# pouyaardehkhani/4DLangSplat

Hardware: AMD Instinct MI355X
Metric: rasterizer fwd+bwd frames/sec @ 2M Gaussians, 1352x1014, 32-ch features (higher is better)
Workload: dtype f32; 1 GPU; S2M synthetic (BASELINE configs[2] per GPU; configs[3] batch split); gaussians=2000000, width=1352, height=1014, channels=32, global_batch=8, parallelism=dp1, pipeline=batched, binning=sort, early_views=2, order_on_side=True, num_rendered_mean=5615889

## Files before the change

4dlangsplat_amd/csrc/binning.hip:

```cpp
#include "lsr_common.h"
#include "lsr_internal.h"

namespace lsr {

__global__ void __launch_bounds__(256) k_emit(const EmitBatch eb) {
    __shared__ uint32_t s_off[4][64];
    __shared__ uint2 s_rc[4][64];
    __shared__ uint32_t s_id[4][64];
    __shared__ EmitSplat s_sp[4][64];
    const EmitView& ev = eb.v[blockIdx.y];
    const int P = eb.P, gx = eb.grid_x, W = eb.W, H = eb.H;
    const uint32_t* __restrict__ order = ev.order;
    const uint32_t* __restrict__ offsets = ev.offsets;
    const uint32_t* __restrict__ counts = ev.counts;
    const uint2* __restrict__ rect_sorted = ev.rect_sorted;
    const float2* __restrict__ xy = ev.xy;
    const float4* __restrict__ conic_o = ev.conic_o;
    uint32_t* __restrict__ keys = ev.keys;
    uint32_t* __restrict__ vals = ev.vals;
    clear_words(ev.clear);
    const int w = threadIdx.x >> 6, lane = threadIdx.x & 63;
    const int base = (blockIdx.x * 4 + w) * 64;
    if (base >= P) return;
    const int r = base + lane;
// ... 20 lines not shown
            if (s_off[w][k + step] <= j) k += step;
        const uint2 rc = s_rc[w][k];
        uint32_t x0, y0, x1, y1;
        rect_unpack(rc, x0, y0, x1, y1);
        const uint32_t wd = x1 - x0;
        const uint32_t loc = j - s_off[w][k];
        uint32_t dx, dy, quads;
        if (rect_small(x0, y0, x1, y1)) {
            const uint32_t map = rect_quad_map(rc);
            uint32_t m = rect_tile_mask(map);
            for (uint32_t i = 0; i < loc; ++i) m &= m - 1u;
            const uint32_t pos = (uint32_t)__builtin_ctz(m);
            dx = pos & 1u;
            dy = pos >> 1;
            const uint32_t sh = 8 * dy + 2 * dx;
            quads = ((map >> sh) & 3u) | (((map >> (sh + 4)) & 3u) << 2);
        } else {
            dy = loc / wd;
            dx = loc - dy * wd;
            quads = emit_quad_mask(s_sp[w][k], (int)(x0 + dx) * LSR_TILE_X, (int)(y0 + dy) * LSR_TILE_Y, W, H);
        }
        const uint32_t tx = x0 + dx, ty = y0 + dy;
        keys[j] = quads ? ty * (uint32_t)gx + tx : 0xFFFFFFFFu;
        vals[j] = s_id[w][k] | (quads << PL_QUAD_SHIFT);
    }
}

void launch_emit_instances(const EmitBatch& eb, int nv, hipStream_t st) {
    if (eb.P == 0 || nv <= 0) return;
    hipLaunchKernelGGL(k_emit, dim3((eb.P + 255) / 256, nv), dim3(256), 0, st, eb);
}

__global__ void __launch_bounds__(256) k_scatter_inst_off(int P, const uint32_t* __restrict__ order,
                                                          const uint32_t* __restrict__ offsets,
                                                          const uint32_t* __restrict__ counts,
                                                          uint32_t* __restrict__ inst_off) {
    const int r = blockIdx.x * blockDim.x + threadIdx.x;
    if (r < P && counts[r] > 0) inst_off[order[r]] = offsets[r];
}

void launch_scatter_inst_off(int P, const uint32_t* order, const uint32_t* offsets, const uint32_t* counts,
                             uint32_t* inst_off, hipStream_t st) {
    if (P == 0) return;
    hipLaunchKernelGGL(k_scatter_inst_off, dim3((P + 255) / 256), dim3(256), 0, st, P, order, offsets, counts,
                       inst_off);
}

}
```

4dlangsplat_amd/csrc/lsr_api.hip:

```cpp
#include <hip/hip_runtime.h>

#include <atomic>
#include <cstdio>
#include <cstring>
#include <mutex>
#include <string>
#include <vector>

#include "../../include/lsr.h"
#include "lsr_common.h"
#include "lsr_internal.h"

namespace {

thread_local std::string g_err;
std::atomic<int32_t> g_caller_api{0};

int fail(int code, const std::string& msg) {
    g_err = msg;
    return code;
}

#define LSR_HIP(expr)                                                                        \
    do {                                                                                     \
// ... 40 lines not shown
    ~PhaseTimer() {
        if (!a || !b) return;
        (void)hipEventRecord(b, st);
        std::lock_guard<std::mutex> l(g_prof.mu);
        g_prof.pending.push_back({phase, a, b});
    }
};

constexpr size_t kAlign = 256;
inline size_t al(size_t x) { return (x + kAlign - 1) / kAlign * kAlign; }

struct Carver {
    char* base;
    size_t off = 0;
    explicit Carver(void* b) : base(static_cast<char*>(b)) {}
    template <typename T>
    T* take(size_t n) {
        T* p = base ? reinterpret_cast<T*>(base + off) : nullptr;
        off += al(n * sizeof(T));
        return p;
    }
};

struct Geom {
    float2* xy;
    float4* conic_o;
    float4* rgbd;
    uint8_t* clamped;
    uint32_t* tiles;
    uint32_t *key_a, *key_b, *val_a, *val_b;
    uint32_t* counts;
    uint32_t* offsets;
    uint32_t* inst_off;
    int* radius;
    uint2* rect;
    uint2* rect_sorted;
    uint32_t* total;
    void* sort_tmp;
    void* scan_tmp;
    float4* acc;
};
Geom carve_geom(void* base, size_t P, size_t* bytes) {
    Carver c(base);
    Geom g;
    g.xy = c.take<float2>(P);
    g.conic_o = c.take<float4>(P);
    g.rgbd = c.take<float4>(P);
    g.clamped = c.take<uint8_t>(P);
    g.tiles = c.take<uint32_t>(P);
    g.key_a = c.take<uint32_t>(P);
    g.key_b = c.take<uint32_t>(P);
    g.val_a = c.take<uint32_t>(P);
    g.val_b = c.take<uint32_t>(P);
    g.counts = c.take<uint32_t>(P);
    g.offsets = c.take<uint32_t>(P);
    g.inst_off = c.take<uint32_t>(P);
    g.radius = c.take<int>(P);
    g.rect = c.take<uint2>(P);
    g.rect_sorted = c.take<uint2>(P);
    g.total = c.take<uint32_t>(4);
    g.sort_tmp = c.take<char>(lsr::radix_temp_bytes(P));
    g.scan_tmp = c.take<char>(lsr::scan_temp_bytes(P));
    g.acc = c.take<float4>(P * (lsr::ACC_PITCH / 4));
    if (bytes) *bytes = c.off;
    return g;
}

struct Binning {
    uint32_t *key_a, *key_b, *val_a, *val_b;
    void* sort_tmp;
    uint32_t* kept;
};
Binning carve_binning(void* base, size_t K, size_t* bytes) {
    Carver c(base);
    Binning b;
    b.key_a = c.take<uint32_t>(K);
    b.key_b = c.take<uint32_t>(K);
    b.val_a = c.take<uint32_t>(K);
    b.val_b = c.take<uint32_t>(K);
    b.sort_tmp = c.take<char>(lsr::radix_temp_bytes(K));
    b.kept = c.take<uint32_t>(4);
    if (bytes) *bytes = c.off;
    return b;
}

struct BinningTb {
    Binning b;
    uint32_t* table;
    uint64_t* tmp;
};
// ... 120 lines not shown
        if (!rules.share_first && !shares(s[v], s[0], rules.share)) return fail(LSR_EINVAL, rules.share_msg);
    }
    return LSR_OK;
}
int need_radii(int32_t n_views, lsr_fwd_out* const* out, int P) {
    for (int v = 0; v < n_views; ++v)
        if (!out[v] || (!out[v]->radii && P > 0)) return fail(LSR_EINVAL, "radii output is required");
    return LSR_OK;
}
int need_workspaces(const void* geom, const void* img, const void* binning, int64_t num_rendered) {
    if (!geom || !img || (num_rendered > 0 && !binning)) return fail(LSR_EINVAL, "workspaces are required");
    return LSR_OK;
}
int need_atomic_grads(const lsr_bwd_in* gin, const char* color_msg, const char* deterministic_msg) {
    if (!gin || !gin->dL_dout_color) return fail(LSR_EINVAL, color_msg);
    if (gin->deterministic) return fail(LSR_EINVAL, deterministic_msg);
    return LSR_OK;
}

void preprocess_shared(lsr::PreprocessArgs& a, const lsr_settings* s, const lsr_fwd_in* in) {
    const int W = s->image_width, H = s->image_height;
    const Grid grid = tile_grid(W, H);
    a.P = in->P; a.M = in->M; a.deg = s->sh_degree; a.W = W; a.H = H;
    a.grid_x = grid.x; a.grid_y = grid.y;
    a.scale_modifier = s->scale_modifier;
    a.means3D = in->means3D; a.scales = in->scales; a.rotations = in->rotations; a.opacities = in->opacities;
    a.shs = in->shs; a.colors_precomp = in->colors_precomp; a.cov3D_precomp = in->cov3D_precomp;
}
void preprocess_view(lsr::PreprocessView& v, const lsr_settings* s, const Geom& g, int* radii) {
    v.tanfovx = s->tanfovx; v.tanfovy = s->tanfovy;
    v.focal_x = focal(s->image_width, s->tanfovx);
    v.focal_y = focal(s->image_height, s->tanfovy);
    v.view = s->viewmatrix; v.proj = s->projmatrix; v.campos = s->campos;
    v.radii = radii; v.radius = g.radius; v.tiles = g.tiles; v.rect = g.rect; v.key = g.key_a; v.xy = g.xy;
    v.conic_o = g.conic_o; v.rgbd = g.rgbd; v.clamped = g.clamped;
    v.order = g.val_a;
    v.rank_counts = g.counts;
    v.acc = g.acc;
    v.clear.p[0] = g.total;
    v.clear.n[0] = 4;
}

uint32_t* mapped_counts(uint32_t* host_counts) {
    void* dptr = nullptr;
    if (hipHostGetDevicePointer(&dptr, host_counts, 0) == hipSuccess && dptr) return static_cast<uint32_t*>(dptr);
    (void)hipGetLastError();
    return nullptr;
}

int scan_counts(int nv, void* const* geom, int P, uint32_t* host_counts, uint32_t* mapped, hipStream_t st, bool debug) {
    lsr::ScanSeg sc[lsr::LSR_MAX_VIEWS] = {};
    const uint32_t* total[lsr::LSR_MAX_VIEWS];
    for (int k = 0; k < nv; ++k) {
        Geom g = carve_geom(geom[k], (size_t)P, nullptr);
        sc[k] = lsr::ScanSeg{g.counts, g.offsets, g.total, reinterpret_cast<uint32_t*>(g.scan_tmp), (size_t)P};
        total[k] = g.total;
        if (mapped) {
            sc[k].host_total = mapped + 2 * k;
            host_counts[2 * k + 1] = 0;
        }
    }
    uint32_t wrote;
    {
        PhaseTimer t(LSR_PHASE_INSTANCE_SCAN, st);
        wrote = lsr::exclusive_scan_batch(sc, nv, st);
    }
    LSR_LAUNCHED("instance scan", st, debug);
    for (int k = 0; k < nv; ++k)
        if (!((wrote >> k) & 1u))
// ... 66 lines not shown
    if (row1 == row0) return LSR_OK;
    for (int v0 = 0; v0 < n_views; v0 += lsr::LSR_MAX_VIEWS) {
        const int nv = std::min(n_views - v0, lsr::LSR_MAX_VIEWS);
        lsr::PreprocessArgs a{};
        preprocess_shared(a, s[v0], in);
        a.nv = nv;
        a.row0 = row0;
        a.P = row1;
        a.counts_tiles = counts_tiles;
        for (int k = 0; k < nv; ++k) {
            Geom g = carve_geom(geom[v0 + k], (size_t)P, nullptr);
            preprocess_view(a.v[k], s[v0 + k], g, out[v0 + k]->radii);
        }
        {
            PhaseTimer t(LSR_PHASE_PREPROCESS, st);
            lsr::launch_preprocess(a, st);
        }
        LSR_LAUNCHED("preprocess", st, s[v0]->debug);
    }
    return LSR_OK;
}

int depth_order_views(int32_t n_views, const lsr_settings* const* s, const lsr_fwd_in* in, void* const* geom,
                      uint32_t* host_counts, uint32_t* mapped, hipStream_t st) {
    const int P = in->P;
    for (int v0 = 0; v0 < n_views; v0 += lsr::LSR_MAX_VIEWS) {
        const int nv = std::min(n_views - v0, lsr::LSR_MAX_VIEWS);
        lsr::SortSeg ss[lsr::LSR_MAX_VIEWS] = {};
        for (int k = 0; k < nv; ++k) {
            Geom g = carve_geom(geom[v0 + k], (size_t)P, nullptr);
            ss[k] = lsr::SortSeg{g.key_a, g.val_a, g.key_b, g.val_b, g.sort_tmp, g.total + 3,
                                 lsr::SortGather{g.rect, g.counts, g.rect_sorted}, (size_t)P};
            ss[k].vals_c = g.offsets;
        }
        {
            PhaseTimer t(LSR_PHASE_DEPTH_SORT, st);
            if (lsr::radix_sort_batch(ss, nv, 0, 32, st) != depth_sort_result_in_b())
                return fail(LSR_EHIP, "internal: depth sort batch or parity");
        }
        LSR_LAUNCHED("depth sort", st, s[v0]->debug);
        int rc = scan_counts(nv, geom + v0, P, host_counts + 2 * v0, mapped ? mapped + 2 * v0 : nullptr, st,
                             s[v0]->debug);
        if (rc) return rc;
    }
    return LSR_OK;
}

int instance_scan_views(int32_t n_views, const lsr_fwd_in* in, void* const* geom, uint32_t* host_counts,
                        uint32_t* mapped, hipStream_t st, bool debug) {
    for (int v0 = 0; v0 < n_views; v0 += lsr::LSR_MAX_VIEWS) {
        int rc = scan_counts(std::min(n_views - v0, lsr::LSR_MAX_VIEWS), geom + v0, in->P, host_counts + 2 * v0,
                             mapped ? mapped + 2 * v0 : nullptr, st, debug);
        if (rc) return rc;
    }
    return LSR_OK;
}
}
}

namespace {
int preprocess_and_order(int32_t n_views, int32_t n_ordered, const lsr_settings* const* s, const lsr_fwd_in* in,
                         lsr_fwd_out* const* out, void* const* geom, uint32_t* host_counts, bool map_counts,
                         hipStream_t st) {
    if (in->P == 0) {
        for (int v = 0; v < 2 * n_ordered; ++v) host_counts[v] = 0;
        return LSR_OK;
// ... 129 lines not shown
    LSR_HIP(hipStreamSynchronize(reinterpret_cast<hipStream_t>(stream)));
    *num_rendered = (int64_t)tot[0];
    return LSR_OK;
}

int lsr_forward_binning(const lsr_settings* s, const lsr_fwd_in* in, void* geom, void* binning, void* img,
                        int64_t num_rendered, lsr_stream_t stream) {
    return lsr_forward_binning_views(1, &s, in, &geom, &binning, &img, &num_rendered, stream);
}

int lsr_forward_binning_views(int32_t n_views, const lsr_settings* const* s, const lsr_fwd_in* in, void* const* geom,
                              void* const* binning, void* const* img, const int64_t* num_rendered,
                              lsr_stream_t stream) {
    const auto emit_and_sort = [](const BinBatch& c, const BinView* bv, int ne) {
        const size_t ntiles = c.ntiles;
        hipStream_t st = c.st;
        lsr::EmitBatch eb{};
        eb.P = c.P; eb.grid_x = c.grid.x; eb.grid_y = c.grid.y; eb.W = c.W; eb.H = c.H;
        lsr::SortSeg ss[lsr::LSR_MAX_VIEWS] = {};
        for (int k = 0; k < ne; ++k) {
            const Geom& g = bv[k].g;
            const Img& m = bv[k].m;
            Binning b = carve_binning(bv[k].binning, bv[k].K, nullptr);
            lsr::EmitView& e = eb.v[k];
            e.order = g.val_a; e.offsets = g.offsets; e.counts = g.counts; e.rect_sorted = g.rect_sorted;
            e.xy = g.xy; e.conic_o = g.conic_o; e.keys = b.key_a; e.vals = b.val_a;
            e.clear.p[0] = reinterpret_cast<uint32_t*>(m.ranges);
            e.clear.n[0] = (uint32_t)(2 * ntiles);
            e.clear.even[0] = 0xFFFFFFFFu;
            e.clear.p[1] = m.tile_max;
            e.clear.n[1] = (uint32_t)ntiles;
            ss[k] = lsr::SortSeg{b.key_a, b.val_a, b.key_b, b.val_b, b.sort_tmp, b.kept,
                                 lsr::SortGather{nullptr, nullptr, nullptr}, bv[k].K, m.ranges, (uint32_t)ntiles};
        }
        {
            PhaseTimer t(LSR_PHASE_EMIT, st);
            lsr::launch_emit_instances(eb, ne, st);
        }
        LSR_LAUNCHED("emit", st, c.debug);
        {
            PhaseTimer t(LSR_PHASE_TILE_SORT, st);
            const int in_b = lsr::radix_sort_batch(ss, ne, 0, tile_bits((int)ntiles), st);
            if (in_b < 0 || (in_b == 1) != tile_sort_in_b((int)ntiles))
                return fail(LSR_EHIP, "internal: tile sort batch or parity");
        }
        LSR_LAUNCHED("tile sort", st, c.debug);
        return LSR_OK;
    };
    return bin_views(n_views, s, in, geom, binning, img, num_rendered, stream, SIZE_MAX, nullptr, emit_and_sort);
}

int lsr_forward_binning_views_tb(int32_t n_views, const lsr_settings* const* s, const lsr_fwd_in* in, void* const* geom,
                                 void* const* binning, void* const* img, const int64_t* num_rendered,
                                 lsr_stream_t stream) {
    const auto bucket = [](const BinBatch& c, const BinView* bv, int ne) {
        lsr::TbBatch tb{};
        tb.P = c.P; tb.grid_x = c.grid.x; tb.grid_y = c.grid.y; tb.W = c.W; tb.H = c.H; tb.ntiles = (int)c.ntiles;
        for (int k = 0; k < ne; ++k) {
            const Geom& g = bv[k].g;
            const Img& m = bv[k].m;
            BinningTb b = carve_binning_tb(bv[k].binning, bv[k].K, (size_t)c.P, c.ntiles, nullptr);
            lsr::TbView& t = tb.v[k];
            t.counts = g.counts; t.offsets = g.offsets; t.rect = g.rect; t.xy = g.xy; t.conic_o = g.conic_o;
            t.depth = g.key_a;
            t.table = b.table;
            t.tile_total = m.tile_order;
// ... 75 lines not shown
    lsr::launch_language_split(P, language_feature, out, reinterpret_cast<hipStream_t>(stream));
    LSR_LAUNCHED("language split", reinterpret_cast<hipStream_t>(stream), false);
    return LSR_OK;
}

int lsr_forward_render(const lsr_settings* s, const lsr_fwd_in* in, lsr_fwd_out* out, void* geom, void* binning,
                       void* img, int64_t num_rendered, lsr_stream_t stream) {
    if (!out || !out->out_color || !out->out_depth) return fail(LSR_EINVAL, "color and depth outputs are required");
    int rc = lsr_forward_binning(s, in, geom, binning, img, num_rendered, stream);
    if (rc) return rc;
    return lsr_forward_composite(s, in, out, geom, binning, img, num_rendered, stream);
}

int lsr_backward(const lsr_settings* s, const lsr_fwd_in* in, const lsr_bwd_in* gin, lsr_bwd_out* gout,
                 const void* geom, const void* binning, const void* img, void* scratch, int64_t num_rendered,
                 int32_t accumulate, lsr_stream_t stream) {
    int rc = check_common(s, in);
    if (rc) return rc;
    if (!gin || !gin->dL_dout_color || !gout) return fail(LSR_EINVAL, "dL_dout_color and outputs are required");
    if (!geom || !img || !scratch || (num_rendered > 0 && !binning)) return fail(LSR_EINVAL, "workspaces are required");
    hipStream_t st = reinterpret_cast<hipStream_t>(stream);
    const int P = in->P, W = s->image_width, H = s->image_height, C = in->C;
    if (P == 0) return LSR_OK;
    const size_t K = (size_t)num_rendered;
    Geom g = carve_geom(const_cast<void*>(geom), (size_t)P, nullptr);
    Binning b = carve_binning(const_cast<void*>(binning), K > 0 ? K : 1, nullptr);
    Img m = carve_img(const_cast<void*>(img), W, H, nullptr);
    const int Ceff = s->include_feature ? C : 0;
    const int recq = lsr::record_floats(Ceff);
    const bool det = gin->deterministic != 0;
    Scratch sc = carve_scratch(scratch, (size_t)P, K > 0 ? K : 1, recq, det, nullptr);
    if (det && K > 0) {
        LSR_HIP(hipMemsetAsync(sc.flags, 0, K, st));
        lsr::launch_scatter_inst_off(P, g.val_a, g.offsets, g.counts, g.inst_off, st);
    }
    if (!det) LSR_HIP(hipMemsetAsync(sc.acc_small, 0, sizeof(float) * lsr::ACC_PITCH * (size_t)P, st));
    if (!accumulate && C > 0 && gout->dL_dlanguage_feature && (!det || Ceff == 0))
        LSR_HIP(hipMemsetAsync(gout->dL_dlanguage_feature, 0, sizeof(float) * (size_t)P * C, st));
    if (K > 0) {
        lsr::RenderBwdArgs r{};
        render_bwd_view(r, s, in, gin, g, b, m);
        r.rec = sc.rec; r.flags = sc.flags; r.recq = recq; r.deterministic = det;
        r.acc_small = sc.acc_small; r.acc_lang = gout->dL_dlanguage_feature;
        {
            PhaseTimer t(LSR_PHASE_RENDER_BWD, st);
            lsr::launch_render_bwd(r, st);
        }
        LSR_LAUNCHED("render backward", st, s->debug);
    }
    lsr::PreprocessBwdArgs a{};
    a.P = P; a.M = in->M; a.deg = s->sh_degree;
    a.tanfovx = s->tanfovx; a.tanfovy = s->tanfovy;
    a.focal_x = focal(W, s->tanfovx);
    a.focal_y = focal(H, s->tanfovy);
    a.scale_modifier = s->scale_modifier;
    a.means3D = in->means3D; a.scales = in->scales; a.rotations = in->rotations; a.shs = in->shs;
    a.cov3D_precomp = in->cov3D_precomp; a.view = s->viewmatrix; a.proj = s->projmatrix; a.campos = s->campos;
    a.tiles = g.tiles;
    a.clamped = g.clamped;
    a.rec = sc.rec; a.flags = sc.flags; a.inst_off = g.inst_off; a.recq = recq;
    a.deterministic = det; a.acc_small = sc.acc_small;
    a.dopacity = gout->dL_dopacity;
    a.dmeans3D = gout->dL_dmeans3D; a.dmeans2D = gout->dL_dmeans2D; a.dcolors = gout->dL_dcolors;
    a.dcov3D = gout->dL_dcov3D; a.dsh = in->shs ? gout->dL_dsh : nullptr; a.dscales = gout->dL_dscales;
    a.drots = gout->dL_drotations;
    {
        PhaseTimer t(LSR_PHASE_PREPROCESS_BWD, st);
// ... 208 lines not shown
```

4dlangsplat_amd/csrc/lsr_internal.h:

```cpp
#pragma once
#include <hip/hip_runtime.h>
#include <stdint.h>

namespace lsr {

constexpr int ACC_PITCH = 16;

struct ClearList {
    uint32_t* p[4];
    uint32_t n[4];
    uint32_t even[4];
};

constexpr int LSR_MAX_VIEWS = 8;
__device__ __forceinline__ void clear_words(const ClearList& c) {
    const uint32_t t = blockIdx.x * blockDim.x + threadIdx.x, stride = gridDim.x * blockDim.x;
#pragma unroll
    for (int k = 0; k < 4; ++k)
        for (uint32_t i = t; i < c.n[k]; i += stride) c.p[k][i] = (i & 1u) ? 0u : c.even[k];
}

__host__ __device__ __forceinline__ uint2 rect_pack(uint32_t x0, uint32_t y0, uint32_t x1, uint32_t y1, uint32_t map) {
    return make_uint2(x0 | y0 << 12 | (map & 0xFFu) << 24, x1 | y1 << 12 | (map >> 8) << 24);
}
__host__ __device__ __forceinline__ void rect_unpack(uint2 r, uint32_t& x0, uint32_t& y0, uint32_t& x1, uint32_t& y1) {
    x0 = r.x & 0xFFFu; y0 = (r.x >> 12) & 0xFFFu; x1 = r.y & 0xFFFu; y1 = (r.y >> 12) & 0xFFFu;
}
__host__ __device__ __forceinline__ uint32_t rect_quad_map(uint2 r) { return (r.x >> 24) | (r.y >> 24) << 8; }
__host__ __device__ __forceinline__ bool rect_small(uint32_t x0, uint32_t y0, uint32_t x1, uint32_t y1) {
    return x1 - x0 <= 2 && y1 - y0 <= 2;
}
__host__ __device__ __forceinline__ uint32_t rect_tile_mask(uint32_t map) {
    return ((map & 0x33u) ? 1u : 0u) | ((map & 0xCCu) ? 2u : 0u) | ((map & 0x3300u) ? 4u : 0u) |
           ((map & 0xCC00u) ? 8u : 0u);
}
__host__ __device__ __forceinline__ uint32_t rect_count(uint2 r) {
    uint32_t x0, y0, x1, y1;
    rect_unpack(r, x0, y0, x1, y1);
    if ((x1 - x0) * (y1 - y0) > 0 && rect_small(x0, y0, x1, y1)) return __builtin_popcount(rect_tile_mask(rect_quad_map(r)));
    return (x1 - x0) * (y1 - y0);
}
__host__ __device__ __forceinline__ uint32_t rect_local_index(uint2 r, uint32_t tx, uint32_t ty) {
    uint32_t x0, y0, x1, y1;
    rect_unpack(r, x0, y0, x1, y1);
    if (rect_small(x0, y0, x1, y1))
        return __builtin_popcount(rect_tile_mask(rect_quad_map(r)) & ((1u << (2 * (ty - y0) + (tx - x0))) - 1u));
    return (ty - y0) * (x1 - x0) + (tx - x0);
}

struct PreprocessView {
    float tanfovx, tanfovy, focal_x, focal_y;
    const float* view;
    const float* proj;
    const float* campos;
    int* radii;
    int* radius;
    uint32_t* tiles;
    uint2* rect;
    uint32_t* key;
    float2* xy;
    float4* conic_o;
    float4* rgbd;
    uint8_t* clamped;
    uint32_t* order;
    uint32_t* rank_counts;
    float4* acc;
    ClearList clear;
};
struct PreprocessArgs {
    int P, M, deg, W, H, grid_x, grid_y, nv;
    int row0;
    int counts_tiles;
    float scale_modifier;
    const float* means3D;
    const float* scales;
    const float* rotations;
    const float* opacities;
    const float* shs;
    const float* colors_precomp;
    const float* cov3D_precomp;
    PreprocessView v[LSR_MAX_VIEWS];
};

struct PreprocessBwdArgs {
    int P, M, deg;
    float tanfovx, tanfovy, focal_x, focal_y, scale_modifier;
    const float* means3D;
    const float* scales;
    const float* rotations;
    const float* shs;
    const float* cov3D_precomp;
    const float* view;
    const float* proj;
    const float* campos;
    const uint32_t* tiles;
    const uint8_t* clamped;
    const float* rec;
// ... 242 lines not shown
void launch_preprocess_bwd(const PreprocessBwdArgs& a, bool accumulate, hipStream_t st);
void launch_reduce_lang(int P, int C, int cpad, int recq, const float* rec, const uint8_t* flags,
                        const uint32_t* inst_off, const uint32_t* tiles, float* dlang, bool accumulate, hipStream_t st);
void launch_mark_visible(int P, const float* means3D, const float* view, uint8_t* present, hipStream_t st);

size_t scan_temp_bytes(size_t n);
void exclusive_scan_u32(const uint32_t* in, uint32_t* out, size_t n, uint32_t* total, void* temp, hipStream_t st);
constexpr int SCAN_SEG_TILES = 4096;
struct ScanSeg {
    const uint32_t* in;
    uint32_t* out;
    uint32_t* total;
    uint32_t* partials;
    size_t n;
    uint32_t* host_total = nullptr;
};
struct ScanBatch { ScanSeg s[LSR_MAX_VIEWS]; };
uint32_t exclusive_scan_batch(const ScanSeg* segs, int nseg, hipStream_t st);
size_t radix_temp_bytes(size_t n);
struct SortGather {
    const uint2* rect;
    uint32_t* counts;
    uint2* rect_sorted;
};
struct SortSeg {
    uint32_t *keys_a, *vals_a, *keys_b, *vals_b;
    void* temp;
    uint32_t* kept;
    SortGather gather;
    size_t n;
    uint2* ranges;
    uint32_t nranges;
    uint32_t* vals_c;
};
struct SortBatch { SortSeg s[LSR_MAX_VIEWS]; };
int radix_sort_batch(const SortSeg* segs, int nseg, int begin_bit, int end_bit, hipStream_t st);
bool radix_sort_pairs(uint32_t* keys_a, uint32_t* vals_a, uint32_t* keys_b, uint32_t* vals_b, size_t n,
                      int begin_bit, int end_bit, void* temp, hipStream_t st, uint32_t* kept = nullptr,
                      const SortGather* gather = nullptr, uint32_t* vals_c = nullptr);

constexpr uint32_t PL_ID_MASK = 0x0FFFFFFFu;
constexpr int PL_QUAD_SHIFT = 28;
struct EmitView {
    const uint32_t* order;
    const uint32_t* offsets;
    const uint32_t* counts;
    const uint2* rect_sorted;
    const float2* xy;
    const float4* conic_o;
    uint32_t* keys;
    uint32_t* vals;
    ClearList clear;
};
struct EmitBatch {
    int P, grid_x, grid_y, W, H;
    EmitView v[LSR_MAX_VIEWS];
};
void launch_emit_instances(const EmitBatch& eb, int nv, hipStream_t st);
void launch_scatter_inst_off(int P, const uint32_t* order, const uint32_t* offsets, const uint32_t* counts,
                             uint32_t* inst_off, hipStream_t st);
struct TbView {
    const uint32_t* counts;
    const uint32_t* offsets;
    const uint2* rect;
    const float2* xy;
    const float4* conic_o;
    const uint32_t* depth;
    uint32_t* table;
    uint32_t* tile_total;
    uint32_t* tile_start;
    uint2* ranges;
    uint64_t* keys;
    uint64_t* tmp;
    uint32_t* words;
    uint32_t* tile_max;
};
struct TbBatch {
    int P, grid_x, grid_y, W, H, ntiles;
    TbView v[LSR_MAX_VIEWS];
};
int tb_blocks(int P);
hipError_t launch_tile_bucket_binning(const TbBatch& tb, int nv, hipStream_t st);

void launch_render_bwd(const RenderBwdArgs& a, hipStream_t st);
void launch_render_fwd_wave_views(const RenderFwdArgs* a, int n, hipStream_t st);
void launch_render_fwd_wave_mfma_views(const RenderFwdArgs* a, int n, hipStream_t st);

}
```

4dlangsplat_amd/csrc/preprocess.hip:

```cpp
#include "lsr_common.h"
#include "lsr_internal.h"

namespace lsr {

struct m3 { float m[3][3]; };

__device__ __forceinline__ m3 mul(const m3& a, const m3& b) {
    m3 o;
#pragma unroll
    for (int c = 0; c < 3; ++c)
#pragma unroll
        for (int r = 0; r < 3; ++r)
            o.m[c][r] = a.m[0][r] * b.m[c][0] + a.m[1][r] * b.m[c][1] + a.m[2][r] * b.m[c][2];
    return o;
}
__device__ __forceinline__ m3 tr(const m3& a) {
    m3 o;
#pragma unroll
    for (int c = 0; c < 3; ++c)
#pragma unroll
        for (int r = 0; r < 3; ++r) o.m[c][r] = a.m[r][c];
    return o;
}
__device__ __forceinline__ m3 quat_R(float4 q) {
// ... 73 lines not shown
#pragma unroll
        for (int k = 0; k < 6; ++k) c3[k] = a.cov3D_precomp[6 * (size_t)i + k];
    } else {
        const float3 s = make_float3(a.scales[3 * i], a.scales[3 * i + 1], a.scales[3 * i + 2]);
        const float4 q = reinterpret_cast<const float4*>(a.rotations)[i];
        cov3d(s, a.scale_modifier, q, c3);
    }
}
template <int MS, int N>
__device__ __forceinline__ void load_sh(const PreprocessArgs& a, int i, float (&shr)[N]) {
    constexpr int M3 = MS * 3;
    const float* src = a.shs + (size_t)i * M3;
    if (M3 % 4 == 0 && (reinterpret_cast<uintptr_t>(src) & 15) == 0) {
#pragma unroll
        for (int q = 0; q < M3 / 4; ++q) {
            const float4 t = reinterpret_cast<const float4*>(src)[q];
            shr[4 * q] = t.x; shr[4 * q + 1] = t.y; shr[4 * q + 2] = t.z; shr[4 * q + 3] = t.w;
        }
    } else {
#pragma unroll
        for (int q = 0; q < M3; ++q) shr[q] = src[q];
    }
}
template <int MS>
__device__ __forceinline__ void load_gauss(const PreprocessArgs& a, int i, GaussIn<MS>& g) {
    g.p = load_mean(a, i);
    g.op = a.opacities[i];
    load_cov3d(a, i, g.c3);
    if constexpr (MS > 0) {
        if (a.shs && !a.colors_precomp) load_sh<MS>(a, i, g.sh);
    }
}

template <int MS, bool PRE>
__device__ __forceinline__ bool preprocess_one(const PreprocessArgs& a, const PreprocessView& v, const GaussIn<MS>& g,
                                               int i) {
    v.radii[i] = 0;
    v.radius[i] = 0;
    v.tiles[i] = 0;
    v.rect[i] = make_uint2(0u, 0u);
    v.clamped[i] = 0;
    if (v.order) v.order[i] = (uint32_t)i;
    if (v.rank_counts) v.rank_counts[i] = 0u;
    if (v.key) v.key[i] = 0xFFFFFFFFu;
    const float3 p = PRE ? g.p : load_mean(a, i);
    const float4 ph = xform4x4(v.proj, p);
    const float3 pv = xform4x3(v.view, p);
    if (pv.z <= 0.2f) return false;
    const float pw = 1.0f / (ph.w + 0.0000001f);
    const float3 pp = make_float3(ph.x * pw, ph.y * pw, ph.z * pw);

    float c3[6];
    if constexpr (PRE) {
#pragma unroll
        for (int k = 0; k < 6; ++k) c3[k] = g.c3[k];
    } else {
        load_cov3d(a, i, c3);
    }
    float3 t = pv;
    const float limx = 1.3f * v.tanfovx, limy = 1.3f * v.tanfovy;
    const float txtz = t.x / t.z, tytz = t.y / t.z;
    t.x = fminf(limx, fmaxf(-limx, txtz)) * t.z;
    t.y = fminf(limy, fmaxf(-limy, tytz)) * t.z;
    m3 J = zero3();
    J.m[0][0] = v.focal_x / t.z; J.m[0][2] = -(v.focal_x * t.x) / (t.z * t.z);
    J.m[1][1] = v.focal_y / t.z; J.m[1][2] = -(v.focal_y * t.y) / (t.z * t.z);
    const m3 T = mul(view_W(v.view), J);
    const m3 V = sym3(c3);
    const m3 A = mul(tr(T), tr(V));
    const m3 cv = mul(A, T);
    const float ca = cv.m[0][0] + 0.3f, cb = cv.m[0][1], cc = cv.m[1][1] + 0.3f;
    const float det = ca * cc - cb * cb;
    if (det == 0.0f) return false;
    const float det_inv = 1.0f / det;
    const float4 conic = make_float4(cc * det_inv, -cb * det_inv, ca * det_inv, PRE ? g.op : a.opacities[i]);
    const float mid = 0.5f * (ca + cc);
    const float l1 = mid + sqrtf(fmaxf(0.1f, mid * mid - det));
// ... 34 lines not shown
            } else {
                load_sh<MS>(a, i, shr);
            }
        }
        const float* sh = MS > 0 ? shr : a.shs + (size_t)i * a.M * 3;
        uint8_t cl = 0;
        const int deg = a.deg;
#pragma unroll
        for (int ch = 0; ch < 3; ++ch) {
#define SHc(k) sh[(k) * 3 + ch]
            float res = SH_C0 * SHc(0);
            if (deg > 0) {
                const float x = dir.x, y = dir.y, z = dir.z;
                res = res - SH_C1 * y * SHc(1) + SH_C1 * z * SHc(2) - SH_C1 * x * SHc(3);
                if (deg > 1) {
                    const float xx = x * x, yy = y * y, zz = z * z, xy = x * y, yz = y * z, xz = x * z;
                    res = res + SH_C2[0] * xy * SHc(4) + SH_C2[1] * yz * SHc(5) +
                          SH_C2[2] * (2.0f * zz - xx - yy) * SHc(6) + SH_C2[3] * xz * SHc(7) +
                          SH_C2[4] * (xx - yy) * SHc(8);
                    if (deg > 2) {
                        res = res + SH_C3[0] * y * (3.0f * xx - yy) * SHc(9) + SH_C3[1] * xy * z * SHc(10) +
                              SH_C3[2] * y * (4.0f * zz - xx - yy) * SHc(11) +
                              SH_C3[3] * z * (2.0f * zz - 3.0f * xx - 3.0f * yy) * SHc(12) +
                              SH_C3[4] * x * (4.0f * zz - xx - yy) * SHc(13) + SH_C3[5] * z * (xx - yy) * SHc(14) +
                              SH_C3[6] * x * (xx - 3.0f * yy) * SHc(15);
                    }
                }
            }
#undef SHc
            res = res + 0.5f;
            cl |= (res < 0.0f ? 1 : 0) << ch;
            rgb[ch] = res < 0.0f ? 0.0f : res;
        }
        v.clamped[i] = cl;
    }
    v.radii[i] = radius;
    v.radius[i] = radius;
    uint32_t qmap = 0;
    if (ntiles > 0 && cmax.x - cmin.x <= 2 && cmax.y - cmin.y <= 2) {
        const EmitSplat es = emit_splat(pix, conic);
        const float ex = emit_margin(es);
        for (int ty = cmin.y; ty < cmax.y; ++ty)
#pragma unroll
            for (int band = 0; band < 2; ++band) {
                bool ok;
                float xmin, xmax;
                emit_band(es, ty * LSR_TILE_Y + 8 * band, a.H, ex, ok, xmin, xmax);
                for (int tx = cmin.x; tx < cmax.x; ++tx)
#pragma unroll
                    for (int col = 0; col < 2; ++col)
                        qmap |= emit_col_hit(es, ok, xmin, xmax, tx * LSR_TILE_X + 8 * col, a.W)
                                    ? 1u << (8 * (ty - cmin.y) + 4 * band + 2 * (tx - cmin.x) + col) : 0u;
            }
    }
    const uint2 rc = rect_pack((uint32_t)cmin.x, (uint32_t)cmin.y, (uint32_t)cmax.x, (uint32_t)cmax.y, qmap);
    v.rect[i] = rc;
    v.tiles[i] = rect_count(rc);
    if (v.rank_counts && a.counts_tiles) v.rank_counts[i] = rect_count(rc);
    if (v.key) v.key[i] = __float_as_uint(pv.z);
    v.xy[i] = pix;
    v.conic_o[i] = conic;
    v.rgbd[i] = make_float4(rgb[0], rgb[1], rgb[2], pv.z);
    return ntiles > 0;
}

__device__ __forceinline__ void zero_acc_rows(float4* acc, bool rect, int i) {
    if (!acc) return;
    const uint64_t m = __ballot(rect);
    if (m == 0) return;
    const int ln = threadIdx.x & 63;
    float4* w = acc + (size_t)(i - ln) * (ACC_PITCH / 4);
#pragma unroll
    for (int q = 0; q < ACC_PITCH / 4; ++q) {
        const int e = q * 64 + ln;
        if ((m >> (e / (ACC_PITCH / 4))) & 1) w[e] = make_float4(0.0f, 0.0f, 0.0f, 0.0f);
    }
}

template <int MS, bool MULTI>
__global__ void __launch_bounds__(256) k_preprocess(PreprocessArgs a) {
    const int i = a.row0 + blockIdx.x * blockDim.x + threadIdx.x;
    GaussIn<MS> g;
    if constexpr (!MULTI) {
        clear_words(a.v[0].clear);
        const bool rect = i < a.P && preprocess_one<MS, false>(a, a.v[0], g, i);
        zero_acc_rows(a.v[0].acc, rect, i);
    } else {
        const bool ok = i < a.P;
        if (ok) load_gauss<MS>(a, i, g);
        for (int k = 0; k < a.nv; ++k) {
            const PreprocessView& v = a.v[k];
            clear_words(v.clear);
            const bool rect = ok && preprocess_one<MS, true>(a, v, g, i);
            zero_acc_rows(v.acc, rect, i);
        }
    }
// ... 628 lines not shown
```

4dlangsplat_amd/csrc/sort.hip:

```cpp
#include "lsr_common.h"
#include "lsr_internal.h"
#include <cstdlib>

namespace lsr {

constexpr int SCAN_ITEMS = 8;
constexpr int SCAN_TILE = 256 * SCAN_ITEMS;

static inline size_t align_up(size_t x, size_t a) { return (x + a - 1) / a * a; }

__device__ __forceinline__ void block_exclusive_scan8(uint32_t (&v)[SCAN_ITEMS], uint32_t* s_wave,
                                                      uint32_t& block_total) {
    const int lane = threadIdx.x & 63, wave = threadIdx.x >> 6;
    uint32_t local = 0;
#pragma unroll
    for (int i = 0; i < SCAN_ITEMS; ++i) { const uint32_t x = v[i]; v[i] = local; local += x; }
    uint32_t inc = local;
#pragma unroll
    for (int o = 1; o < 64; o <<= 1) {
        const uint32_t t = __shfl_up(inc, o);
        if (lane >= o) inc += t;
    }
    if (lane == 63) s_wave[wave] = inc;
    __syncthreads();
// ... 426 lines not shown
        const int v = e ? std::atoi(e) : 0;
        return (v == 4 || v == 8 || v == 16) ? v : 16;
    }();
    return dg;
}
static void launch_rts_scan(const SortBatch& bt, int ns, int p, int items, int in_b, int nbits, hipStream_t st) {
    switch (scan_dg()) {
        case 4: hipLaunchKernelGGL(k_rts_scan<4>, dim3(RDX / 4, ns), dim3(256), 0, st, bt, p, items, in_b, nbits); break;
        case 8: hipLaunchKernelGGL(k_rts_scan<8>, dim3(RDX / 8, ns), dim3(256), 0, st, bt, p, items, in_b, nbits); break;
        default: hipLaunchKernelGGL(k_rts_scan<16>, dim3(RDX / 16, ns), dim3(256), 0, st, bt, p, items, in_b, nbits); break;
    }
}

template <int IT>
__global__ void __launch_bounds__(256) k_rts_scatter(const SortBatch b, int pass, int in_b, int shift, int nbits_h,
                                                     int last_h) {
    __shared__ uint32_t s_key[(256 * IT)];
    __shared__ uint32_t s_val[(256 * IT)];
    __shared__ uint32_t s_wcnt[4][RDX];
    __shared__ uint32_t s_gbase[RDX];
    __shared__ uint32_t s_lbase[RDX];
    __shared__ uint32_t s_wave[4];
    const SortSeg& sg = b.s[blockIdx.y];
    const size_t nbi = rts_blocks(sg.n, IT);
    const uint32_t bid = blockIdx.x;
    if (bid >= nbi) return;
    const PassDesc pd = pass_desc(sg, pass, in_b, shift, nbits_h, last_h);
    if (!pd.active) return;
    const uint32_t* __restrict__ keys_in = keys_of(sg, pd.src);
    const uint32_t* __restrict__ vals_in = vals_of(sg, pd.src);
    uint32_t* __restrict__ keys_out = keys_of_w(sg, pd.dst);
    uint32_t* __restrict__ vals_out = vals_of_w(sg, pd.dst);
    const int drop = sg.kept && pass == 0;
    uint32_t* kept_out = drop ? sg.kept : nullptr;
    const uint32_t* __restrict__ totals = rts_totals(sg, pass);
    const uint32_t* __restrict__ offs = rts_rows(sg, pass, nbi);
    const SortGather gather = pd.last ? sg.gather : SortGather{nullptr, nullptr, nullptr};
    const int tid = threadIdx.x, wave = tid >> 6, lane = tid & 63;
    const int nd = 1 << pd.nbits;
#pragma unroll
    for (int w = 0; w < 4; ++w) {
        s_wcnt[w][tid] = 0;
        s_wcnt[w][tid + 256] = 0;
    }
    const size_t n = rts_n(sg.n, sg.kept && pass > 0 ? sg.kept : nullptr);
    __syncthreads();
    const uint32_t mask = (uint32_t)nd - 1u;
    const uint64_t lt = lanemask_lt();
    const size_t base = (size_t)bid * (256 * IT) + (size_t)wave * (64 * IT);
    uint32_t key[IT], val[IT], rank[IT];
#pragma unroll
    for (int r = 0; r < IT; ++r) {
        const size_t idx = base + (size_t)r * 64 + lane;
        const bool valid = idx < n;
        key[r] = valid ? keys_in[idx] : 0u;
        val[r] = valid ? vals_in[idx] : 0u;
    }
    const int da = 2 * tid, db = 2 * tid + 1;
    const uint32_t pre_a = da < nd ? offs[(size_t)bid * RDX + da] : 0u, pre_b = db < nd ? offs[(size_t)bid * RDX + db] : 0u;
    const uint32_t hc_a = da < nd ? totals[da] : 0u, hc_b = db < nd ? totals[db] : 0u;
#pragma unroll
    for (int r = 0; r < IT; ++r) {
        const bool valid = base + (size_t)r * 64 + lane < n && !(drop && key[r] == 0xFFFFFFFFu);
        const uint32_t d = ((key[r] - pd.kbase) >> pd.shift) & mask;
        const uint64_t peers = match_digit(d, valid, pd.nbits);
        const uint32_t before = s_wcnt[wave][d];
        const uint32_t pr = (uint32_t)__popcll(peers & lt);
        rank[r] = before + pr;
        __builtin_amdgcn_wave_barrier();
        if (valid && pr == 0) s_wcnt[wave][d] = before + (uint32_t)__popcll(peers);
        __builtin_amdgcn_wave_barrier();
    }
    __syncthreads();
    uint32_t tot_a, tot_b;
    {
        const uint32_t a0 = s_wcnt[0][da], a1 = s_wcnt[1][da], a2 = s_wcnt[2][da], a3 = s_wcnt[3][da];
        const uint32_t b0 = s_wcnt[0][db], b1 = s_wcnt[1][db], b2 = s_wcnt[2][db], b3 = s_wcnt[3][db];
        tot_a = a0 + a1 + a2 + a3;
        tot_b = b0 + b1 + b2 + b3;
        s_wcnt[0][da] = 0; s_wcnt[1][da] = a0; s_wcnt[2][da] = a0 + a1; s_wcnt[3][da] = a0 + a1 + a2;
        s_wcnt[0][db] = 0; s_wcnt[1][db] = b0; s_wcnt[2][db] = b0 + b1; s_wcnt[3][db] = b0 + b1 + b2;
    }
    const uint32_t dstart_a = block_excl_scan256(hc_a + hc_b, s_wave);
    const uint32_t lbase_a = block_excl_scan256(tot_a + tot_b, s_wave);
    s_lbase[da] = lbase_a;
    s_lbase[db] = lbase_a + tot_a;
    s_gbase[da] = dstart_a + pre_a - lbase_a;
    s_gbase[db] = dstart_a + hc_a + pre_b - (lbase_a + tot_a);
    if (tid == 255) {
// ... 9 lines not shown
            const uint32_t d = ((key[r] - pd.kbase) >> pd.shift) & mask;
            const uint32_t pos = s_lbase[d] + s_wcnt[wave][d] + rank[r];
            s_key[pos] = key[r];
            s_val[pos] = val[r];
        }
    }
    __syncthreads();
    if (gather.rect) {
        uint2 rc[IT];
        uint32_t vv[IT], dd[IT];
#pragma unroll
        for (int r = 0; r < IT; ++r) {
            const int i = tid + 256 * r;
            const bool ok = i < ntile;
            const uint32_t k = s_key[ok ? i : 0], v = s_val[ok ? i : 0];
            vv[r] = v;
            dd[r] = s_gbase[((k - pd.kbase) >> pd.shift) & mask] + (uint32_t)i;
            rc[r] = ok ? gather.rect[v] : make_uint2(0u, 0u);
        }
#pragma unroll
        for (int r = 0; r < IT; ++r) {
            if (tid + 256 * r < ntile) {
                vals_out[dd[r]] = vv[r];
                gather.rect_sorted[dd[r]] = rc[r];
                gather.counts[dd[r]] = rect_count(rc[r]);
            }
        }
        return;
    }
    uint2* __restrict__ ranges = pd.last ? sg.ranges : nullptr;
    for (int i = tid; i < ntile; i += 256) {
        const uint32_t k = s_key[i];
        const uint32_t dst = s_gbase[((k - pd.kbase) >> pd.shift) & mask] + (uint32_t)i;
        keys_out[dst] = k;
        vals_out[dst] = s_val[i];
        if (ranges && k < sg.nranges) {
            if (i == 0 || s_key[i - 1] != k) atomicMin(&ranges[k].x, dst);
            if (i == ntile - 1 || s_key[i + 1] != k) atomicMax(&ranges[k].y, dst + 1u);
        }
    }
}

static size_t os_blocks(size_t n) { return (n + OS_TILE - 1) / OS_TILE; }

size_t radix_temp_bytes(size_t n) {
    return RTS_ROWS_OFF + align_up(4 * os_blocks(n) * RDX * 4, 256);
}

int radix_sort_batch(const SortSeg* segs, int nseg, int begin_bit, int end_bit, hipStream_t st) {
    SortBatch bt{};
    int ns = 0;
    size_t nmax = 0;
    for (int i = 0; i < nseg; ++i)
        if (segs[i].n > 0) { bt.s[ns++] = segs[i]; nmax = std::max(nmax, segs[i].n); }
    if (ns == 0 || end_bit <= begin_bit) return 0;
    for (int i = 1; i < ns; ++i)
        if ((bt.s[i].vals_c == nullptr) != (bt.s[0].vals_c == nullptr)) return -1;
    if (bt.s[0].vals_c && (begin_bit != 0 || end_bit != 32)) return -1;
    static const int depth_items = [] {
        const char* e = std::getenv("LSR_DEPTH_ITEMS");
        return e && std::atoi(e) == 8 ? OS_ITEMS : 12;
    }();
    const int items = nmax > ((size_t)4 << 20) ? 12 : (bt.s[0].vals_c ? depth_items : OS_ITEMS);
    const unsigned nbi = (unsigned)((nmax + 256 * items - 1) / (256 * items));
    auto pass = [&](int p, int in_b, int shift, int nbits, int last) {
        if (items == 12)
            hipLaunchKernelGGL(k_rts_count<12>, dim3(nbi, ns), dim3(256), 0, st, bt, p, in_b, shift, nbits);
// ... 34 lines not shown
```

Measured before the change: 992.7 frames/s.

## Trim redundant global writes in preprocess and sort passes

Drops the duplicate radius buffer and the per-Gaussian order array written in preprocess. The depth sort's first pass now generates identity values from the index instead of reading them. The tile sort skips writing keys on its final pass when they are unused. Preprocess now only stores xy/conic/rgbd for live Gaussians, and the inst_off scatter falls back to the identity when no sort ran. This cuts memory traffic, but correctness now depends on stale xy/conic data never being read for culled Gaussians and on the ranked flag being set correctly.

```diff
diff --git a/4dlangsplat_amd/csrc/binning.hip b/4dlangsplat_amd/csrc/binning.hip
--- a/4dlangsplat_amd/csrc/binning.hip
+++ b/4dlangsplat_amd/csrc/binning.hip
@@ -76,17 +76,20 @@
 }
 
 __global__ void __launch_bounds__(256) k_scatter_inst_off(int P, const uint32_t* __restrict__ order,
+                                                          const uint32_t* __restrict__ ranked,
                                                           const uint32_t* __restrict__ offsets,
                                                           const uint32_t* __restrict__ counts,
                                                           uint32_t* __restrict__ inst_off) {
     const int r = blockIdx.x * blockDim.x + threadIdx.x;
-    if (r < P && counts[r] > 0) inst_off[order[r]] = offsets[r];
+    if (r >= P || counts[r] == 0) return;
+    const uint32_t id = *ranked ? order[r] : (uint32_t)r;
+    if (id < (uint32_t)P) inst_off[id] = offsets[r];
 }
 
-void launch_scatter_inst_off(int P, const uint32_t* order, const uint32_t* offsets, const uint32_t* counts,
-                             uint32_t* inst_off, hipStream_t st) {
+void launch_scatter_inst_off(int P, const uint32_t* order, const uint32_t* ranked, const uint32_t* offsets,
+                             const uint32_t* counts, uint32_t* inst_off, hipStream_t st) {
     if (P == 0) return;
-    hipLaunchKernelGGL(k_scatter_inst_off, dim3((P + 255) / 256), dim3(256), 0, st, P, order, offsets, counts,
+    hipLaunchKernelGGL(k_scatter_inst_off, dim3((P + 255) / 256), dim3(256), 0, st, P, order, ranked, offsets, counts,
                        inst_off);
 }
 
diff --git a/4dlangsplat_amd/csrc/lsr_api.hip b/4dlangsplat_amd/csrc/lsr_api.hip
--- a/4dlangsplat_amd/csrc/lsr_api.hip
+++ b/4dlangsplat_amd/csrc/lsr_api.hip
@@ -96,7 +96,6 @@
     uint32_t* counts;
     uint32_t* offsets;
     uint32_t* inst_off;
-    int* radius;
     uint2* rect;
     uint2* rect_sorted;
     uint32_t* total;
@@ -119,7 +118,6 @@
     g.counts = c.take<uint32_t>(P);
     g.offsets = c.take<uint32_t>(P);
     g.inst_off = c.take<uint32_t>(P);
-    g.radius = c.take<int>(P);
     g.rect = c.take<uint2>(P);
     g.rect_sorted = c.take<uint2>(P);
     g.total = c.take<uint32_t>(4);
@@ -306,9 +304,8 @@
     v.focal_x = focal(s->image_width, s->tanfovx);
     v.focal_y = focal(s->image_height, s->tanfovy);
     v.view = s->viewmatrix; v.proj = s->projmatrix; v.campos = s->campos;
-    v.radii = radii; v.radius = g.radius; v.tiles = g.tiles; v.rect = g.rect; v.key = g.key_a; v.xy = g.xy;
+    v.radii = radii; v.tiles = g.tiles; v.rect = g.rect; v.key = g.key_a; v.xy = g.xy;
     v.conic_o = g.conic_o; v.rgbd = g.rgbd; v.clamped = g.clamped;
-    v.order = g.val_a;
     v.rank_counts = g.counts;
     v.acc = g.acc;
     v.clear.p[0] = g.total;
@@ -441,6 +438,7 @@
             ss[k] = lsr::SortSeg{g.key_a, g.val_a, g.key_b, g.val_b, g.sort_tmp, g.total + 3,
                                  lsr::SortGather{g.rect, g.counts, g.rect_sorted}, (size_t)P};
             ss[k].vals_c = g.offsets;
+            ss[k].iota_vals = 1;
         }
         {
             PhaseTimer t(LSR_PHASE_DEPTH_SORT, st);
@@ -636,6 +634,7 @@
             e.clear.n[1] = (uint32_t)ntiles;
             ss[k] = lsr::SortSeg{b.key_a, b.val_a, b.key_b, b.val_b, b.sort_tmp, b.kept,
                                  lsr::SortGather{nullptr, nullptr, nullptr}, bv[k].K, m.ranges, (uint32_t)ntiles};
+            ss[k].keys_dead = 1;
         }
         {
             PhaseTimer t(LSR_PHASE_EMIT, st);
@@ -777,7 +776,7 @@
     Scratch sc = carve_scratch(scratch, (size_t)P, K > 0 ? K : 1, recq, det, nullptr);
     if (det && K > 0) {
         LSR_HIP(hipMemsetAsync(sc.flags, 0, K, st));
-        lsr::launch_scatter_inst_off(P, g.val_a, g.offsets, g.counts, g.inst_off, st);
+        lsr::launch_scatter_inst_off(P, g.val_a, g.total + 3, g.offsets, g.counts, g.inst_off, st);
     }
     if (!det) LSR_HIP(hipMemsetAsync(sc.acc_small, 0, sizeof(float) * lsr::ACC_PITCH * (size_t)P, st));
     if (!accumulate && C > 0 && gout->dL_dlanguage_feature && (!det || Ceff == 0))
diff --git a/4dlangsplat_amd/csrc/lsr_internal.h b/4dlangsplat_amd/csrc/lsr_internal.h
--- a/4dlangsplat_amd/csrc/lsr_internal.h
+++ b/4dlangsplat_amd/csrc/lsr_internal.h
@@ -54,7 +54,6 @@
     const float* proj;
     const float* campos;
     int* radii;
-    int* radius;
     uint32_t* tiles;
     uint2* rect;
     uint32_t* key;
@@ -62,7 +61,6 @@
     float4* conic_o;
     float4* rgbd;
     uint8_t* clamped;
-    uint32_t* order;
     uint32_t* rank_counts;
     float4* acc;
     ClearList clear;
@@ -371,6 +369,8 @@
     uint2* ranges;
     uint32_t nranges;
     uint32_t* vals_c;
+    int iota_vals;
+    int keys_dead;
 };
 struct SortBatch { SortSeg s[LSR_MAX_VIEWS]; };
 int radix_sort_batch(const SortSeg* segs, int nseg, int begin_bit, int end_bit, hipStream_t st);
@@ -396,8 +396,8 @@
     EmitView v[LSR_MAX_VIEWS];
 };
 void launch_emit_instances(const EmitBatch& eb, int nv, hipStream_t st);
-void launch_scatter_inst_off(int P, const uint32_t* order, const uint32_t* offsets, const uint32_t* counts,
-                             uint32_t* inst_off, hipStream_t st);
+void launch_scatter_inst_off(int P, const uint32_t* order, const uint32_t* ranked, const uint32_t* offsets,
+                             const uint32_t* counts, uint32_t* inst_off, hipStream_t st);
 struct TbView {
     const uint32_t* counts;
     const uint32_t* offsets;
diff --git a/4dlangsplat_amd/csrc/preprocess.hip b/4dlangsplat_amd/csrc/preprocess.hip
--- a/4dlangsplat_amd/csrc/preprocess.hip
+++ b/4dlangsplat_amd/csrc/preprocess.hip
@@ -129,17 +129,21 @@
     }
 }
 
+struct Projected {
+    int radius = 0;
+    uint32_t tiles = 0u;
+    uint2 rect = make_uint2(0u, 0u);
+    uint8_t clamped = 0;
+    uint32_t key = 0xFFFFFFFFu;
+    bool rects = false;
+    float2 xy;
+    float4 conic_o;
+    float4 rgbd;
+};
+
 template <int MS, bool PRE>
-__device__ __forceinline__ bool preprocess_one(const PreprocessArgs& a, const PreprocessView& v, const GaussIn<MS>& g,
-                                               int i) {
-    v.radii[i] = 0;
-    v.radius[i] = 0;
-    v.tiles[i] = 0;
-    v.rect[i] = make_uint2(0u, 0u);
-    v.clamped[i] = 0;
-    if (v.order) v.order[i] = (uint32_t)i;
-    if (v.rank_counts) v.rank_counts[i] = 0u;
-    if (v.key) v.key[i] = 0xFFFFFFFFu;
+__device__ __forceinline__ bool project_one(const PreprocessArgs& a, const PreprocessView& v, const GaussIn<MS>& g,
+                                            int i, Projected& o) {
     const float3 p = PRE ? g.p : load_mean(a, i);
     const float4 ph = xform4x4(v.proj, p);
     const float3 pv = xform4x3(v.view, p);
@@ -240,10 +244,9 @@
             cl |= (res < 0.0f ? 1 : 0) << ch;
             rgb[ch] = res < 0.0f ? 0.0f : res;
         }
-        v.clamped[i] = cl;
-    }
-    v.radii[i] = radius;
-    v.radius[i] = radius;
+        o.clamped = cl;
+    }
+    o.radius = radius;
     uint32_t qmap = 0;
     if (ntiles > 0 && cmax.x - cmin.x <= 2 && cmax.y - cmin.y <= 2) {
         const EmitSplat es = emit_splat(pix, conic);
@@ -261,15 +264,33 @@
                                     ? 1u << (8 * (ty - cmin.y) + 4 * band + 2 * (tx - cmin.x) + col) : 0u;
             }
     }
-    const uint2 rc = rect_pack((uint32_t)cmin.x, (uint32_t)cmin.y, (uint32_t)cmax.x, (uint32_t)cmax.y, qmap);
-    v.rect[i] = rc;
-    v.tiles[i] = rect_count(rc);
-    if (v.rank_counts && a.counts_tiles) v.rank_counts[i] = rect_count(rc);
-    if (v.key) v.key[i] = __float_as_uint(pv.z);
-    v.xy[i] = pix;
-    v.conic_o[i] = conic;
-    v.rgbd[i] = make_float4(rgb[0], rgb[1], rgb[2], pv.z);
-    return ntiles > 0;
+    o.rect = rect_pack((uint32_t)cmin.x, (uint32_t)cmin.y, (uint32_t)cmax.x, (uint32_t)cmax.y, qmap);
+    o.tiles = rect_count(o.rect);
+    o.key = __float_as_uint(pv.z);
+    o.xy = pix;
+    o.conic_o = conic;
+    o.rgbd = make_float4(rgb[0], rgb[1], rgb[2], pv.z);
+    o.rects = ntiles > 0;
+    return true;
+}
+
+template <int MS, bool PRE>
+__device__ __forceinline__ bool preprocess_one(const PreprocessArgs& a, const PreprocessView& v, const GaussIn<MS>& g,
+                                               int i) {
+    Projected o;
+    const bool live = project_one<MS, PRE>(a, v, g, i, o);
+    v.radii[i] = o.radius;
+    v.tiles[i] = o.tiles;
+    v.rect[i] = o.rect;
+    v.clamped[i] = o.clamped;
+    if (v.rank_counts) v.rank_counts[i] = a.counts_tiles ? o.tiles : 0u;
+    if (v.key) v.key[i] = o.key;
+    if (live) {
+        v.xy[i] = o.xy;
+        v.conic_o[i] = o.conic_o;
+        v.rgbd[i] = o.rgbd;
+    }
+    return o.rects;
 }
 
 __device__ __forceinline__ void zero_acc_rows(float4* acc, bool rect, int i) {
diff --git a/4dlangsplat_amd/csrc/sort.hip b/4dlangsplat_amd/csrc/sort.hip
--- a/4dlangsplat_amd/csrc/sort.hip
+++ b/4dlangsplat_amd/csrc/sort.hip
@@ -482,6 +482,8 @@
     uint32_t* __restrict__ keys_out = keys_of_w(sg, pd.dst);
     uint32_t* __restrict__ vals_out = vals_of_w(sg, pd.dst);
     const int drop = sg.kept && pass == 0;
+    const bool iota = sg.iota_vals && pass == 0;
+    const bool put_keys = !(pd.last && sg.keys_dead);
     uint32_t* kept_out = drop ? sg.kept : nullptr;
     const uint32_t* __restrict__ totals = rts_totals(sg, pass);
     const uint32_t* __restrict__ offs = rts_rows(sg, pass, nbi);
@@ -504,7 +506,7 @@
         const size_t idx = base + (size_t)r * 64 + lane;
         const bool valid = idx < n;
         key[r] = valid ? keys_in[idx] : 0u;
-        val[r] = valid ? vals_in[idx] : 0u;
+        val[r] = !valid ? 0u : iota ? (uint32_t)idx : vals_in[idx];
     }
     const int da = 2 * tid, db = 2 * tid + 1;
     const uint32_t pre_a = da < nd ? offs[(size_t)bid * RDX + da] : 0u, pre_b = db < nd ? offs[(size_t)bid * RDX + db] : 0u;
@@ -580,7 +582,7 @@
     for (int i = tid; i < ntile; i += 256) {
         const uint32_t k = s_key[i];
         const uint32_t dst = s_gbase[((k - pd.kbase) >> pd.shift) & mask] + (uint32_t)i;
-        keys_out[dst] = k;
+        if (put_keys) keys_out[dst] = k;
         vals_out[dst] = s_val[i];
         if (ranges && k < sg.nranges) {
             if (i == 0 || s_key[i - 1] != k) atomicMin(&ranges[k].x, dst);
```

New measurement: 981.9 frames/s. -1.1%, worse.
